# chengl7-lab/scape

Hardware: AMD Instinct MI355X
Metric: UTR regions/sec (infer_pa EM to convergence), 50k UTRs x 2k reads synthetic (higher is better)
Workload: dtype f64; 1 GPU; 50k-UTR synthetic stream x 2000 reads, K=1..10 x 10 restarts; step = one resident batch of 512 UTRs per GPU; reads_per_utr=2000, k_cap=10, n_frag_max=1469, re_run_mode=False, rng_mode=per_utr, parallelism=utr-shard x1

## Files before the change

### scape_amd/csrc/em_lockstep.inc

```

#define MT_RB 1
#define MT_ROWS (64 * MT_RB)
#define MT_NC 32
#define MT_PITCH (MT_NC + 2)
#define MT_VPITCH (MT_NC + 2)
#define MT_MAXJ 64
#ifndef EM_DEPTH
#define EM_DEPTH 3
#endif
static_assert(EM_DEPTH >= 1 && EM_DEPTH <= 8, "column slots per job");
#ifndef MT_DV1
#define MT_DV1 1
#endif

#ifndef MT_DEEP
#define MT_DEEP 2
#endif
#define CNT_SLAB 4
#define CNT_EXEC (4 + 64)
#define CNT_MSTEP_TENSOR (4 + 2 * 64)
#define CNT_MSTEP_VREQ (4 + 3 * 64)
#define CNT_MSTEP_VUNI (4 + 4 * 64)
static_assert(MT_ROWS == TILE_ROWS, "tile height must match k_tile_extent / the host tables");
static_assert(MT_MAXJ <= 64, "the per-pass job setup gives one job to each lane of one wavefront");

struct EmState {
    int32_t *ia, *ib, *sia, *sib;
    double *ws, *slw;
    double *lb, *ell;
    int32_t *nlb, *status;
    unsigned long long *pend;
    int32_t *rd_k, *rd_lo, *rd_hi, *rd_m;
    int32_t *rd_n0, *rd_n1;
    double *rd_lw, *rd_sv;
    double *rd_fl;
    double *V;
    double *Vsuf;
    const int64_t *voff;
    double *pt_score;
    int32_t *pt_row;
    const int64_t *ptoff;
};

__device__ __forceinline__ double d_wave_allsum(double v) {
#pragma unroll
    for (int off = 32; off > 0; off >>= 1) v += __shfl_xor(v, off, 64);
    return v;
}

#ifndef ESTEP_EXP_GROUP
#define ESTEP_EXP_GROUP 1
#endif
struct EstepNext {
    int status;
    int nlb;
    int pub_k;
    int k_next;
};

template <int CA, int CX, int NW = 1>
__device__ __forceinline__ EstepNext estep_body(
    const UtrDesc *__restrict__ descs, const DevParams &P, const double *__restrict__ cnt,
    const double *__restrict__ M, int kmax, const int32_t *__restrict__ job_utr,
    const int32_t *__restrict__ job_K, const int32_t *__restrict__ job_fixed,
    const int32_t *__restrict__ a_in, const int32_t *__restrict__ b_in,
    const double *__restrict__ ws_in, const int8_t *__restrict__ k_arr, const EmState &S,
    int32_t *__restrict__ a_out, int32_t *__restrict__ b_out, double *__restrict__ ws_out,
    double *__restrict__ bic_out, int32_t *__restrict__ nlb_out, double *__restrict__ lb_out,
    unsigned long long *__restrict__ counters, int launch, int slot, int depth, int job, int lane, int status,
    unsigned long long *s_roff, double *s_lwc, double *s_wsum ,
    const double2 *s_exptab , int wave = 0, double *s_xz = nullptr ,
    double *s_tot = nullptr ) {
    constexpr int CMAX = CA;
#ifdef ESTEP_STAMPS
    const unsigned long long st0 = __builtin_amdgcn_s_memtime();
#define ESTEP_STAMP(v) const unsigned long long v = __builtin_amdgcn_s_memtime()
#else
#define ESTEP_STAMP(v)
#endif
    const bool lead = (NW == 1) || wave == 0;
    const int nround = P.nround, B = P.B;
    const int u_job = job_utr[job];
    const int K = (CX > 0) ? CX - 1 : job_K[job], C = K + 1;
    const bool fixed = job_fixed[job] != 0;
    int32_t *ia = S.ia + (size_t)job * kmax, *ib = S.ib + (size_t)job * kmax;
    int32_t *sia = S.sia + (size_t)job * kmax, *sib = S.sib + (size_t)job * kmax;
    double *ws = S.ws + (size_t)job * (kmax + 1), *slw = S.slw + (size_t)job * (kmax + 1);
    const bool r0 = launch == 0 && slot == 0;
    const bool resolve = slot == 0 && launch > 0;
    const size_t col0 = (size_t)job * depth, col = col0 + slot;
    int pre_m[EM_DEPTH], pre_lo[EM_DEPTH], pre_hi[EM_DEPTH], pre_k[EM_DEPTH];
    int64_t pre_ptoff[EM_DEPTH];
    double pre_fl[EM_DEPTH];
    bool rdm = false;
#pragma unroll
    for (int q = 0; q < EM_DEPTH; ++q) {
        const bool on = resolve && q < depth;
        pre_m[q] = on ? S.rd_m[col0 + q] : 0;
        pre_lo[q] = on ? S.rd_lo[col0 + q] : 0;
        pre_hi[q] = on ? S.rd_hi[col0 + q] : 0;
        pre_k[q] = on ? S.rd_k[col0 + q] : 0;
        pre_ptoff[q] = on ? S.ptoff[col0 + q] : 0;
        pre_fl[q] = on ? S.rd_fl[col0 + q] : 0.0;
        rdm = rdm || pre_m[q] != 0;
    }
    const int64_t pre_voff = S.voff[col];
    const int k_lane = (lane < nround) ? (int)k_arr[(size_t)job * nround + lane] : 0;
    const double lb_prev = r0 ? SENT : S.lb[job];
    const int nlb_prev = r0 ? 0 : S.nlb[job];
    auto k_of_round = [&](int i) {
        const int ii = min(i, nround - 1);
        return (nround <= 64) ? __shfl(k_lane, ii, 64) : (int)k_arr[(size_t)job * nround + ii];
    };
    const int k_now = k_of_round(nlb_prev);
    const int k_next = __builtin_amdgcn_readfirstlane(k_of_round(nlb_prev + 1));
    double my_ws = 0.0, my_slw = 0.0;
    int my_ia = 0, my_ib = 0, my_sia = 0, my_sib = 0;
    if (lane < C) {
        my_ws = r0 ? ws_in[(size_t)job * (kmax + 1) + lane] : ws[lane];
        if (!r0) my_slw = slw[lane];
        if (lane < K) {
            my_ia = r0 ? a_in[(size_t)job * kmax + lane] : ia[lane];
            my_ib = r0 ? b_in[(size_t)job * kmax + lane] : ib[lane];
            my_sia = r0 ? my_ia : sia[lane];
// ... 34 lines not shown
                ia[lane] = sia[lane] = my_ia;
                ib[lane] = sib[lane] = my_ib;
            }
        }
        if (lane == 0) {
            S.lb[job] = SENT;
            S.nlb[job] = 0;
            S.ell[job] = 0.0;
        }
    }
    int upd_k[EM_DEPTH], upd_a[EM_DEPTH], upd_b[EM_DEPTH];
#pragma unroll
    for (int q = 0; q < EM_DEPTH; ++q) {
        upd_k[q] = -1;
        upd_a[q] = upd_b[q] = 0;
        if (pre_m[q]) {
            double best = pt_best[q];
            int best_r = pt_best_r[q];
#pragma unroll
            for (int off = 32; off > 0; off >>= 1) {
                const double ob = __shfl_xor(best, off, 64);
                const int orr = __shfl_xor(best_r, off, 64);
                if (ob > best || (ob == best && orr < best_r)) {
                    best = ob;
                    best_r = orr;
                }
            }
            upd_k[q] = pre_k[q];
            upd_a[q] = best_r / B;
            upd_b[q] = best_r - upd_a[q] * B;
            if (lead && lane == 0) {
                ia[upd_k[q]] = upd_a[q];
                ib[upd_k[q]] = upd_b[q];
            }
            if (lane == upd_k[q]) {
                my_ia = upd_a[q];
                my_ib = upd_b[q];
            }
        }
    }
    if (slot == 0 && lead && lane == 0 && (r0 || rdm))
        for (int q = 0; q < depth; ++q) S.rd_m[col0 + q] = 0;
    auto cur_ia = [&](int i) {
        int v = ia[i];
#pragma unroll
        for (int q = 0; q < EM_DEPTH; ++q) v = (i == upd_k[q]) ? upd_a[q] : v;
        return v;
    };
    auto cur_ib = [&](int i) {
        int v = ib[i];
#pragma unroll
        for (int q = 0; q < EM_DEPTH; ++q) v = (i == upd_k[q]) ? upd_b[q] : v;
        return v;
    };

    if (status == 1 || nlb_prev >= nround) {
        if (lead && lane == 0) {
            const int n_lb = S.nlb[job];
            bic_out[job] = d_bic(S.ell[job], K, N);
            nlb_out[job] = n_lb;
            int idx[CMAX];
            for (int i = 0; i < K; ++i) idx[i] = i;
            for (int i = 1; i < K; ++i) {
                const int v = idx[i];
                int j = i - 1;
                while (j >= 0 && cur_ia(idx[j]) > cur_ia(v)) {
                    idx[j + 1] = idx[j];
                    --j;
                }
                idx[j + 1] = v;
            }
            for (int i = 0; i < K; ++i) {
                a_out[(size_t)job * kmax + i] = cur_ia(idx[i]);
                b_out[(size_t)job * kmax + i] = cur_ib(idx[i]);
                ws_out[(size_t)job * (kmax + 1) + i] = ws[idx[i]];
            }
            ws_out[(size_t)job * (kmax + 1) + K] = ws[K];
            for (int i = K; i < kmax; ++i) {
                a_out[(size_t)job * kmax + i] = -1;
                b_out[(size_t)job * kmax + i] = -1;
                ws_out[(size_t)job * (kmax + 1) + i + 1] = 0.0;
            }
            S.status[job] = 2;
            atomicAdd(&counters[0], (unsigned long long)n_lb);
            atomicAdd(&counters[2], (unsigned long long)n_lb * (unsigned long long)N * (unsigned long long)C);
        }
        return EstepNext{2, nlb_prev, -1, 0};
    }

    if (lead && lane == 0) atomicAdd(&counters[CNT_EXEC + (job & 63)], 1ull);
    const int k = k_now;
    const double wk_old = __shfl(my_ws, k, 64);
    const double slw_k = d_logw(wk_old);
    const int sia_k = (k < K) ? __shfl(my_ia, k, 64) : 0;
    const int sib_k = (k < K) ? __shfl(my_ib, k, 64) : 0;
    const int ia_km1 = __shfl(my_ia, max(k - 1, 0), 64), ia_kp1 = __shfl(my_ia, min(k + 1, 63), 64);
    if (lead && lane == 0) {
        slw[k] = slw_k;
        if (k < K) {
            sia[k] = sia_k;
            sib[k] = sib_k;
        }
    }
    if (lead && lane < CMAX) {
        const int c = lane;
        int sa = 0, sb = 0;
        double lw_c = 0.0;
        if (c < C) {
            if (c == k) {
                lw_c = slw_k;
                sa = sia_k;
                sb = sib_k;
            } else {
                lw_c = my_slw;
                sa = my_sia;
                sb = my_sib;
            }
        }
        s_roff[c] = (c < K) ? ((unsigned long long)sa * B + sb) * Np : 0ull;
        s_lwc[c] = (c < K) ? lw_c : lw_c + d.unif_ll;
    }
    __syncthreads();
    double *Vj = S.V + pre_voff;

    ESTEP_STAMP(st1);
    double tot_w[CMAX], t_sumk = 0.0, t_ell = 0.0, t_ent = 0.0;
    int nz_lo = 0x7fffffff, nz_hi = -1;
    bool mod = false;
    if constexpr (NW == 1) {
        for (int pass = 0; pass < 2; ++pass) {
    #pragma unroll
            for (int c = 0; c < CMAX; ++c) s_wsum[c * 64 + lane] = 0.0;
            double sumk = 0.0, ell = 0.0, ent = 0.0;
            nz_lo = 0x7fffffff;
            nz_hi = -1;
            double mcur[CMAX], ccur = 0.0;
            auto fetch = [&](int n, double (&m)[CMAX], double &cn) {
                const bool ok = n < N;
                cn = ok ? cu[n] : 0.0;
    #pragma unroll
                for (int c = 0; c < CMAX; ++c) m[c] = (ok && c < K) ? Mu[s_roff[c] + n] : 0.0;
            };
            fetch(lane, mcur, ccur);
    #pragma unroll
            for (int c = 0; c < CMAX; ++c) asm volatile("" : "+v"(mcur[c]));
            asm volatile("" : "+v"(ccur));
            for (int n = lane; n < Np; n += 64) {
                double mnext[CMAX], cnext;
                fetch(n + 64, mnext, cnext);
                double vkn = 0.0;
                if (n < N) {
                    const double cn = ccur;
                    auto lzv = [&](int c) { return (c < K) ? s_lwc[c] + mcur[c] : s_lwc[c]; };
                    double mx = 0.0;
    #pragma unroll
                    for (int c = 0; c < CMAX; ++c) {
                        if (c < C) {
                            const double v = lzv(c);
                            mx = (c == 0 || v > mx) ? v : mx;
                        }
                    }
                    double z[CMAX];
                    unsigned long long live = 0ull;
#if ESTEP_EXP_GROUP >= 2
    #pragma unroll
                    for (int c = 0; c < CMAX; c += ESTEP_EXP_GROUP) {
// ... 300 lines not shown
        S.lb[job] = lb_new;
        S.status[job] = status_new;
        S.rd_m[col] = has_m ? 1 : 0;
        if (has_m) {
            const int lo = (k == 0) ? 0 : ia_km1;
            const int hi = (k == K - 1) ? d.T - 1 : ia_kp1;
            S.rd_k[col] = k;
            S.rd_lo[col] = lo * B;
            S.rd_hi[col] = (hi + 1) * B;
            S.rd_lw[col] = d_logw(wk_new);
            S.rd_sv[col] = sv;
            S.rd_fl[col] = d_logw(wk_new) * sv + SENT * v_total;
            S.rd_n0[col] = (nz_hi >= 0) ? nz_lo : 0;
            S.rd_n1[col] = (nz_hi >= 0) ? nz_hi + 1 : 0;
            atomicAdd(&counters[CNT_SLAB + (job & 63)], (unsigned long long)(hi + 1 - lo) * B * (unsigned long long)N);
        }
    }
#ifdef ESTEP_STAMPS
    if (NW == 1 && lane == 0) {
        const unsigned long long st5 = __builtin_amdgcn_s_memtime();
        unsigned long long *sp = counters + 4 + 5 * 64;
        atomicAdd(&sp[0], st1 - st0);
        atomicAdd(&sp[1], st2 - st1);
        atomicAdd(&sp[2], st3 - st2);
        atomicAdd(&sp[3], st4 - st3);
        atomicAdd(&sp[4], st5 - st4);
        atomicAdd(&sp[7], 1ull);
    }
#endif
#undef ESTEP_STAMP
    return EstepNext{status_new, nlb_prev + 1, has_m ? k : -1, k_next};
}

#define ESTEP_ARGS(ROUND, STATUS) descs, P, cnt, M, kmax, job_utr, job_K, job_fixed, a_in, b_in, ws_in, k_arr, S, a_out, \
                   b_out, ws_out, bic_out, nlb_out, lb_out, counters, ROUND, slot, depth, job, lane, STATUS, s_roff, s_lwc, s_wsum, s_exptab
#define ESTEP_CASE(C, ROUND, STATUS) \
    case C: nx = estep_body<C, C, ESTEP_NW>(ESTEP_ARGS(ROUND, STATUS) ESTEP_EXTRA); break;
#define ESTEP_DISPATCH(CM, ROUND, STATUS)                                                         \
    do {                                                                                          \
        if constexpr (CM <= 16) {                                                                 \
            const int c_exact = job_K[job] + 1;                                                   \
            if constexpr (CM >= 16) {                                                             \
                if (c_exact > 12) {                                                               \
                    switch (c_exact) {                                                            \
                        ESTEP_CASE(13, ROUND, STATUS) ESTEP_CASE(14, ROUND, STATUS)               \
                        ESTEP_CASE(15, ROUND, STATUS)                                             \
                        default: nx = estep_body<16, 16, ESTEP_NW>(ESTEP_ARGS(ROUND, STATUS) ESTEP_EXTRA); break;            \
                    }                                                                             \
                    break;                                                                        \
                }                                                                                 \
            }                                                                                     \
            if constexpr (CM >= 12) {                                                             \
                if (c_exact > 8) {                                                                \
                    switch (c_exact) {                                                            \
                        ESTEP_CASE(9, ROUND, STATUS) ESTEP_CASE(10, ROUND, STATUS)                \
                        ESTEP_CASE(11, ROUND, STATUS)                                             \
                        default: nx = estep_body<12, 12, ESTEP_NW>(ESTEP_ARGS(ROUND, STATUS) ESTEP_EXTRA); break;            \
                    }                                                                             \
                    break;                                                                        \
                }                                                                                 \
            }                                                                                     \
            if constexpr (CM >= 8) {                                                              \
                if (c_exact > 4) {                                                                \
                    switch (c_exact) {                                                            \
                        ESTEP_CASE(5, ROUND, STATUS) ESTEP_CASE(6, ROUND, STATUS)                 \
                        ESTEP_CASE(7, ROUND, STATUS)                                              \
                        default: nx = estep_body<8, 8, ESTEP_NW>(ESTEP_ARGS(ROUND, STATUS) ESTEP_EXTRA); break;              \
                    }                                                                             \
                    break;                                                                        \
                }                                                                                 \
            }                                                                                     \
            switch (c_exact) {                                                                    \
                ESTEP_CASE(1, ROUND, STATUS) ESTEP_CASE(2, ROUND, STATUS) ESTEP_CASE(3, ROUND, STATUS) \
                default: nx = estep_body<4, 4, ESTEP_NW>(ESTEP_ARGS(ROUND, STATUS) ESTEP_EXTRA); break;                      \
            }                                                                                     \
        } else {                                                                                  \
            nx = estep_body<CM, 0, ESTEP_NW>(ESTEP_ARGS(ROUND, STATUS) ESTEP_EXTRA);                                       \
        }                                                                                         \
    } while (0)

__host__ __device__ inline bool em_run_ahead_stops(int status, int nlb, int nround, int k_next, unsigned long long pend) {
    return status != 0 || nlb >= nround || (pend & (7ull << k_next)) != 0ull;
}
#define ESTEP_NW 1
#ifndef ESTEP_WPS
#define ESTEP_WPS 3
#endif
#define ESTEP_EXTRA
template <int CMAX>
__global__ __launch_bounds__(64, (CMAX > 12 ? 2 : ESTEP_WPS)) void k2_estep(
    const UtrDesc *__restrict__ descs, DevParams P, const double *__restrict__ cnt,
    const double *__restrict__ M, int kmax, const int32_t *__restrict__ job_utr,
    const int32_t *__restrict__ job_K, const int32_t *__restrict__ job_fixed,
    const int32_t *__restrict__ a_in, const int32_t *__restrict__ b_in,
    const double *__restrict__ ws_in, const int8_t *__restrict__ k_arr, EmState S,
    int32_t *__restrict__ a_out, int32_t *__restrict__ b_out, double *__restrict__ ws_out,
    double *__restrict__ bic_out, int32_t *__restrict__ nlb_out, double *__restrict__ lb_out,
    unsigned long long *__restrict__ counters, int launch, int slot, int depth, const int32_t *__restrict__ job_list,
    int n_jobs) {
    const int chunk = (n_jobs + 7) >> 3;
    const int jidx = (int)(blockIdx.x & 7) * chunk + (int)(blockIdx.x >> 3);
    if (jidx >= n_jobs) return;
    const int job = job_list[jidx];
    const int lane = threadIdx.x;
    const int status = (launch == 0 && slot == 0) ? 0 : S.status[job];
    if (status == 2) return;
    unsigned long long pend = 0ull;
    if (slot > 0) {
        pend = S.pend[job];
        if (!(pend & 1ull)) return;
        pend &= ~1ull;
    }
    __shared__ unsigned long long s_roff[CMAX];
    __shared__ double s_lwc[CMAX];
    __shared__ double s_wsum[CMAX * 64];
    __shared__ double2 s_exptab[128];
    d_load_exptab(s_exptab, lane, 64);
    EstepNext nx;
    ESTEP_DISPATCH(CMAX, launch, status);
    if (depth > 1 && lane == 0) {
        if (nx.pub_k >= 0) pend |= 2ull << nx.pub_k;
        const bool stop = em_run_ahead_stops(nx.status, nx.nlb, P.nround, nx.k_next, pend) || job_fixed[job] != 0;
        S.pend[job] = pend | (stop ? 0ull : 1ull);
    }
}

template <int CMAX>
__global__ __launch_bounds__(64, (CMAX > 12 ? 2 : 3)) void k2_estep_all_rounds(
    const UtrDesc *__restrict__ descs, DevParams P, const double *__restrict__ cnt,
    const double *__restrict__ M, int kmax, const int32_t *__restrict__ job_utr,
    const int32_t *__restrict__ job_K, const int32_t *__restrict__ job_fixed,
    const int32_t *__restrict__ a_in, const int32_t *__restrict__ b_in,
    const double *__restrict__ ws_in, const int8_t *__restrict__ k_arr, EmState S,
    int32_t *__restrict__ a_out, int32_t *__restrict__ b_out, double *__restrict__ ws_out,
    double *__restrict__ bic_out, int32_t *__restrict__ nlb_out, double *__restrict__ lb_out,
    unsigned long long *__restrict__ counters, const int32_t *__restrict__ job_list, int n_jobs) {
    const int chunk = (n_jobs + 7) >> 3;
    const int jidx = (int)(blockIdx.x & 7) * chunk + (int)(blockIdx.x >> 3);
    if (jidx >= n_jobs) return;
    const int job = job_list[jidx];
    const int lane = threadIdx.x;
    __shared__ unsigned long long s_roff[CMAX];
    __shared__ double s_lwc[CMAX];
    __shared__ double s_wsum[CMAX * 64];
    __shared__ double2 s_exptab[128];
    d_load_exptab(s_exptab, lane, 64);
    for (int round = 0; round <= P.nround; ++round) {
        const int status = (round == 0) ? 0 : S.status[job];
        if (status == 2) return;
        constexpr int slot = 0, depth = 1;
        EstepNext nx;
        ESTEP_DISPATCH(CMAX, round, status);
        (void)nx;
        __threadfence();
        __syncthreads();
    }
}
#undef ESTEP_NW
#undef ESTEP_EXTRA
#define ESTEP_NW 4
#define ESTEP_EXTRA , wave, s_xz, s_tot
template <int CMAX>
__global__ __launch_bounds__(256, 1) void k2_estep_cs(
    const UtrDesc *__restrict__ descs, DevParams P, const double *__restrict__ cnt,
    const double *__restrict__ M, int kmax, const int32_t *__restrict__ job_utr,
    const int32_t *__restrict__ job_K, const int32_t *__restrict__ job_fixed,
// ... 313 lines not shown
```

### scape_amd/csrc/scape_hip.hip

```cpp
#include <hip/hip_runtime.h>

#include <algorithm>
#include <atomic>
#include <cmath>
#include <cstdint>
#include <cstdio>
#include <cstdlib>
#include <cstring>
#include <memory>
#include <string>
#include <type_traits>
#include <chrono>
#include <utility>
#include <vector>

#include "scape_hip.h"

#define SENT SCAPE_SENT
#define PI_REF 3.141592653589793
#define PITCH 16
#define TILE_ROWS 64

static thread_local std::string g_err;
static int fail(const std::string &msg) {
// ... 557 lines not shown
            if (c < C) {
                lz[c] = (c < K) ? slw[c] + Mu[roff[c] + n] : slw[c] + d.unif_ll;
                mx = (c == 0 || lz[c] > mx) ? lz[c] : mx;
            } else {
                lz[c] = 0.0;
            }
        }
#pragma unroll
        for (int c = 0; c < CMAX; ++c) z[c] = (c < C) ? d_exp_nonpos((lz[c] - mx) * cn, s_exptab) : 0.0;
        const double s = d_np_sum<CMAX>(z, C);
        int best = 0;
        double bz = 0.0;
#pragma unroll
        for (int c = 0; c < CMAX; ++c) {
            const double zc = z[c] / s;
            if (c < C && (c == 0 || zc > bz)) {
                bz = zc;
                best = c;
            }
        }
        labels[d.bin_off + n] = best;
    }
}

struct DevBuf {
    void *p = nullptr;
    size_t cap = 0;
    DevBuf() = default;
    DevBuf(const DevBuf &) = delete;
    DevBuf &operator=(const DevBuf &) = delete;
    ~DevBuf() { release(); }
    int ensure(size_t bytes) {
        if (bytes <= cap && p) return 0;
        const bool regrow = p != nullptr || (bytes > ((size_t)1 << 30) && bytes <= ((size_t)48 << 30));
        if (p) {
            (void)hipFree(p);
            p = nullptr;
            cap = 0;
        }
        if (bytes == 0) bytes = 16;
        size_t want = regrow ? bytes + bytes / 8 : bytes;
        if (hipMalloc(&p, want) != hipSuccess) {
            (void)hipGetLastError();
            p = nullptr;
            want = bytes;
            HIPCHK(hipMalloc(&p, want));
        }
        cap = want;
        return 0;
    }
    void release() {
        if (p) (void)hipFree(p);
        p = nullptr;
        cap = 0;
    }
    template <typename T>
    T *as() const {
        return reinterpret_cast<T *>(p);
    }
};
static_assert(!std::is_copy_constructible<DevBuf>::value && !std::is_copy_assignable<DevBuf>::value,
              "a copy of a DevBuf would free its memory twice");

struct StreamDrain {
    hipStream_t stream;
    bool armed;
    explicit StreamDrain(hipStream_t s, bool a = true) : stream(s), armed(a) {}
    StreamDrain(const StreamDrain &) = delete;
    StreamDrain &operator=(const StreamDrain &) = delete;
    int wait() { armed = false; HIPCHK(hipStreamSynchronize(stream)); return 0; }
    ~StreamDrain() { if (armed) (void)hipStreamSynchronize(stream); }
};

struct EventPair {
    hipEvent_t a, b;
};

struct ReportState;

struct EmBufs {
    DevBuf ia, ib, sia, sib, ws, slw, lb, ell, nlb, status, pend, rd_k, rd_lo, rd_hi, rd_m, rd_n0, rd_n1, rd_lw, rd_sv, rd_fl, V, Vsuf,
        voff, pt_score, pt_row, ptoff;
    DevBuf ujoff, ujlist, active, elist, dbg;
    int ensure(size_t nj, size_t nc, size_t kmax, size_t n_utr, size_t vtot, size_t pttot) {
        return ia.ensure(nj * kmax * 4) || ib.ensure(nj * kmax * 4) || sia.ensure(nj * kmax * 4) || sib.ensure(nj * kmax * 4) ||
               ws.ensure(nj * (kmax + 1) * 8) || slw.ensure(nj * (kmax + 1) * 8) || lb.ensure(nj * 8) || ell.ensure(nj * 8) ||
               nlb.ensure(nj * 4) || status.ensure(nj * 4) || pend.ensure(nj * 8) || rd_k.ensure(nc * 4) || rd_lo.ensure(nc * 4) ||
               rd_hi.ensure(nc * 4) || rd_m.ensure(nc * 4) || rd_n0.ensure(nc * 4) || rd_n1.ensure(nc * 4) ||
               rd_lw.ensure(nc * 8) || rd_sv.ensure(nc * 8) || rd_fl.ensure(nc * 8) || V.ensure(vtot * 8) || Vsuf.ensure((vtot / 16 + nc + 1) * 8) ||
               voff.ensure(nc * 8) || pt_score.ensure(pttot * 8) || pt_row.ensure(pttot * 4) || ptoff.ensure(nc * 8) ||
               ujoff.ensure((n_utr + 1) * 8) || ujlist.ensure(nc * 4) || active.ensure(n_utr * 4) || elist.ensure(nj * 4);
    }
    EmState state() const {
        return EmState{ia.as<int32_t>(), ib.as<int32_t>(), sia.as<int32_t>(), sib.as<int32_t>(), ws.as<double>(), slw.as<double>(),
                       lb.as<double>(), ell.as<double>(), nlb.as<int32_t>(), status.as<int32_t>(), pend.as<unsigned long long>(),
                       rd_k.as<int32_t>(),
                       rd_lo.as<int32_t>(), rd_hi.as<int32_t>(), rd_m.as<int32_t>(), rd_n0.as<int32_t>(), rd_n1.as<int32_t>(),
                       rd_lw.as<double>(), rd_sv.as<double>(), rd_fl.as<double>(), V.as<double>(), Vsuf.as<double>(), voff.as<int64_t>(),
                       pt_score.as<double>(), pt_row.as<int32_t>(), ptoff.as<int64_t>()};
    }
};

static int to_dev(hipStream_t s, const DevBuf &d, const void *src, size_t bytes) {
    HIPCHK(hipMemcpyAsync(d.p, src, bytes, hipMemcpyHostToDevice, s));
    return 0;
}
static int to_host(hipStream_t s, void *dst, const DevBuf &d, size_t bytes) {
    HIPCHK(hipMemcpyAsync(dst, d.p, bytes, hipMemcpyDeviceToHost, s));
    return 0;
}

struct JobBufs {
    DevBuf utr, K, fixed, a, b, ws, karr, ao, bo, wso, bic, nlb, lb, sel, lbsel;
};
struct LabelBufs {
    DevBuf utr, K, a, b, ws, labels;
};

struct BatchShape {
    int n_utr = 0, T_max = 0, Np_max = 0, W_max = 1, tiles_max_all = 1;
    int64_t n_bins = 0;
    std::vector<UtrDesc> h_desc;
    size_t at_total = 0, m_total = 0, tiles_total = 0, n_theta_total = 0, mlog_total = 0, n_logbins = 0;
    bool pb_slide = false;
};
struct BatchPlan : BatchShape {
    std::vector<int32_t> loglist, logbin_utr;
};

struct BatchState : BatchShape {
    DevParams prm;
    bool loaded = false, built = false;
    bool build_unchecked = false;
    int pb_form = 0;
    int last_em_jobs = 0;
    DevBuf d_x, d_l, d_r, d_pa, d_cnt, d_theta, d_desc, d_loglist, d_AT, d_V, d_M, d_tile_nend;
    DevBuf d_tbi, d_tbG, d_tbpm, d_mlog, d_logbin;
    JobBufs job;
    LabelBufs lab;
    EmBufs em;
};

#define N_COUNTERS (4 + 5 * 64 + 16 + 48)
struct scape_hip_ctx {
    int device = 0;
    std::atomic<bool> busy{false};
    hipStream_t stream = nullptr;
    char name[256] = {0};
    std::unique_ptr<BatchState> batch;
    DevBuf d_err, d_counters;
    std::vector<EventPair> ev[6];
    double ms_acc[6] = {0, 0, 0, 0, 0, 0};
    int n_acc[6] = {0, 0, 0, 0, 0, 0};
    unsigned long long h_counters[3] = {0, 0, 0};
    unsigned long long h_traffic[4] = {0, 0, 0, 0};
    ReportState *rep = nullptr;
};

static int ev_begin(scape_hip_ctx *c, int which) {
    EventPair e;
    HIPCHK(hipEventCreate(&e.a));
    HIPCHK(hipEventCreate(&e.b));
    HIPCHK(hipEventRecord(e.a, c->stream));
    c->ev[which].push_back(e);
    return 0;
}
static int ev_end(scape_hip_ctx *c, int which) {
    HIPCHK(hipEventRecord(c->ev[which].back().b, c->stream));
    return 0;
}
static int ev_collect(scape_hip_ctx *c) {
    HIPCHK(hipStreamSynchronize(c->stream));
    const bool trace = getenv("SCAPE_HIP_ROUND_TRACE") != nullptr;
    for (int w = 0; w < 6; ++w) {
        int i = 0;
        for (auto &e : c->ev[w]) {
            float ms = 0;
            HIPCHK(hipEventElapsedTime(&ms, e.a, e.b));
            if (trace && w >= 4) fprintf(stderr, "[trace] kind %d launch %d %.4f ms\n", w, i, ms);
            ++i;
            c->ms_acc[w] += ms;
            c->n_acc[w] += 1;
// ... 94 lines not shown
    const dim3 by_alpha((unsigned)(((b.n_utr + 7) / 8) * 8 * b.T_max));
    if (ch.form == 0) {
#ifdef SCAPE_HIP_TOOLS
        const char *pe = getenv("SCAPE_HIP_PB_PROBE");
        const int probe = pe ? atoi(pe) : 0;
#else
        const int probe = 0;
#endif
        if (b.prm.B <= 16)
            hipLaunchKernelGGL(k_phase_b<16>, by_alpha, dim3(256), ch.lds, c->stream, desc, b.prm, r, pa, theta, loglist, AT, V, M,
                               ch.Wmax, all_log, c->d_err.as<int>(), b.n_utr, b.T_max, tile_nend, probe);
        else
            hipLaunchKernelGGL(k_phase_b<1>, by_alpha, dim3(256), ch.lds, c->stream, desc, b.prm, r, pa, theta, loglist, AT, V, M,
                               ch.Wmax, all_log, c->d_err.as<int>(), b.n_utr, b.T_max, tile_nend, probe);
        HIPCHK(hipGetLastError());
        return 0;
    }
    const bool slide = ch.form == 2;
    hipLaunchKernelGGL(k_pb_tables<16>, dim3((unsigned)b.T_max, (unsigned)b.n_utr), dim3(PB_TAB_THREADS), ch.lds_t, c->stream, desc,
                       b.prm, theta, ch.Wmax, ch.WP, tbi, tbG, tbpm, c->d_err.as<int>(), b.T_max, slide ? nullptr : loglist, AT, M, mlog,
                       tile_nend);
    HIPCHK(hipGetLastError());
    if (slide) {
        if (b.n_logbins) {
            hipLaunchKernelGGL(k_pb_logcol, dim3((unsigned)b.n_logbins), dim3(256), ch.lds_c, c->stream, desc, b.prm, theta, loglist,
                               b.d_logbin.as<int32_t>(), AT, tbi, tbG, M, mlog, tile_nend, ch.Wmax);
            HIPCHK(hipGetLastError());
        }
        const int blocks_max = (b.Np_max + 63) / 64;
        hipLaunchKernelGGL(k_pb_slide, dim3((unsigned)(((b.n_utr + 7) / 8) * 8 * blocks_max)), dim3(256), ch.lds_s, c->stream, desc,
                           b.prm, r, pa, loglist, V, M, mlog, ch.WP, tbi, tbpm, b.n_utr, blocks_max, tile_nend);
    } else {
        hipLaunchKernelGGL(k_phase_b_lin, by_alpha, dim3(256), ch.lds_l, c->stream, desc, b.prm, r, pa, loglist, V, M, mlog, ch.WP, tbi,
                           tbpm, b.n_utr, b.T_max, tile_nend);
    }
    HIPCHK(hipGetLastError());
    return 0;
}

static int check_err_flag(scape_hip_ctx *c, const char *what) {
    int flag = 0;
    HIPCHK(hipMemcpyAsync(&flag, c->d_err.p, sizeof(int), hipMemcpyDeviceToHost, c->stream));
    HIPCHK(hipStreamSynchronize(c->stream));
    if (flag) return fail(std::string(what) + ": device-side consistency check failed (flag " + std::to_string(flag) + ")");
    return 0;
}

static int finish_build(scape_hip_ctx *c) {
    BatchState *b = c->batch.get();
    if (!b || !b->build_unchecked) return 0;
    b->build_unchecked = false;
    b->built = check_err_flag(c, "batch_build") == 0;
    return !b->built;
}

using EstepClasses = std::integer_sequence<int, 4, 8, 12, 16, 24, 32, 64>;
using WideClasses = std::integer_sequence<int, 4, 8, 12, 16>;
using LabelClasses = std::integer_sequence<int, 8, 16, 32, 64>;

template <int... Cs>
constexpr int last_class(std::integer_sequence<int, Cs...>) {
    int last = 0;
    ((last = Cs), ...);
    return last;
}
static_assert(last_class(EstepClasses{}) == SCAPE_MAX_K + 1 && last_class(LabelClasses{}) == SCAPE_MAX_K + 1,
              "the largest class holds the largest kmax a call may have");
constexpr int WIDE_MAX_COLUMNS = last_class(WideClasses{});

template <int... Cs, typename F>
static bool with_column_class(std::integer_sequence<int, Cs...>, int columns, F &&f) {
    return ((columns <= Cs && (f(std::integral_constant<int, Cs>()), true)) || ...);
}

struct EmPlan {
    std::vector<int64_t> ujoff, voff, ptoff;
    std::vector<int32_t> ujlist, active, elist;
    size_t vtot = 0, pttot = 0;
    int depth = 1;
    int tiles_max = 1, max_cols_utr = 1;
    bool any_m = false;
};

static EmPlan em_plan(const std::vector<UtrDesc> &h_desc, int B, size_t nj, const int32_t *job_utr, const int32_t *job_fixed,
                      bool size_order, int depth) {
    EmPlan p;
    const int n_utr = (int)h_desc.size();
    p.depth = depth;
    p.ujoff.assign(n_utr + 1, 0);
    p.ujlist.resize(nj * depth);
    for (size_t j = 0; j < nj; ++j) p.ujoff[job_utr[j] + 1] += depth;
    for (int u = 0; u < n_utr; ++u) p.ujoff[u + 1] += p.ujoff[u];
    {
        std::vector<int64_t> fill(p.ujoff.begin(), p.ujoff.end() - 1);
        for (size_t j = 0; j < nj; ++j)
            for (int q = 0; q < depth; ++q) p.ujlist[fill[job_utr[j]]++] = (int32_t)(j * depth + q);
    }
    for (int u = 0; u < n_utr; ++u)
        if (p.ujoff[u + 1] > p.ujoff[u]) p.active.push_back(u);
    if (size_order)
        std::stable_sort(p.active.begin(), p.active.end(), [&](int32_t a, int32_t b) {
            const UtrDesc &da = h_desc[a], &db = h_desc[b];
            return (int64_t)da.T * da.Np > (int64_t)db.T * db.Np;
        });
    const int n_active = (int)p.active.size();
    for (int u : p.active) {
        p.max_cols_utr = std::max<int>(p.max_cols_utr, (int)(p.ujoff[u + 1] - p.ujoff[u]));
        p.tiles_max = std::max(p.tiles_max, (h_desc[u].T * B + MT_ROWS - 1) / MT_ROWS);
    }
    p.voff.resize(nj * depth);
    p.ptoff.resize(nj * depth);
    for (size_t j = 0; j < nj; ++j) {
        const UtrDesc &d = h_desc[job_utr[j]];
        for (int q = 0; q < depth; ++q) {
            p.voff[j * depth + q] = (int64_t)p.vtot;
            p.ptoff[j * depth + q] = (int64_t)p.pttot;
            p.vtot += (size_t)d.Np;
            p.pttot += (size_t)((d.T * B + MT_ROWS - 1) / MT_ROWS);
        }
        p.any_m = p.any_m || job_fixed[j] == 0;
    }
    p.elist.reserve(nj);
    auto jobs_of = [&](int u) {
        for (int64_t q = p.ujoff[u]; q < p.ujoff[u + 1]; q += depth) p.elist.push_back(p.ujlist[q] / depth);
    };
    if (size_order && n_active >= 8) {
        for (int x = 0; x < 8; ++x)
            for (int k = x; k < n_active; k += 8) jobs_of(p.active[k]);
    } else {
        for (int u = 0; u < n_utr; ++u) jobs_of(u);
    }
    return p;
}

struct EmSwitches {
    bool size_order, debug, fine, mstep_v2, mstep_v3;
    int split_maxtiles, wide_maxjobs;
    int depth;
};
static EmSwitches em_switches() {
    const char *env_m = getenv("SCAPE_HIP_MSTEP"), *env_r = getenv("SCAPE_HIP_SPLIT_MAXTILES"), *env_w = getenv("SCAPE_HIP_WIDE_MAXJOBS");
    EmSwitches s;
    s.size_order = !getenv("SCAPE_HIP_NO_SIZE_ORDER");
    s.debug = getenv("SCAPE_HIP_DEBUG") != nullptr;
    s.fine = getenv("SCAPE_HIP_ROUND_TIMING") != nullptr;
    s.mstep_v2 = env_m && strcmp(env_m, "v2") == 0;
    s.mstep_v3 = env_m && strcmp(env_m, "v3") == 0;
    s.split_maxtiles = env_r ? atoi(env_r) : 1024;
    s.wide_maxjobs = env_w ? atoi(env_w) : 1024;
    const char *env_d = getenv("SCAPE_HIP_EM_DEPTH");
    s.depth = std::min(EM_DEPTH, std::max(1, env_d ? atoi(env_d) : EM_DEPTH));
    return s;
}

struct EmKernels {
    bool wide;
    bool job_split;
    bool ring_mstep;
    bool multi_mstep;
};
static bool em_wide(const EmSwitches &sw, int n_jobs, int kmax) {
    const bool wide = n_jobs <= sw.wide_maxjobs && kmax + 1 <= WIDE_MAX_COLUMNS;
    return wide;
}

static int em_depth(const std::vector<UtrDesc> &h_desc, int B, const EmSwitches &sw, int n_jobs, int kmax, const int32_t *job_utr,
                    const int32_t *job_fixed) {
    bool any_m = false;
    size_t v1 = 0, pt1 = 0;
    std::vector<int> per_utr(h_desc.size(), 0);
    int max_jobs_utr = 1;
    for (int j = 0; j < n_jobs; ++j) {
        const UtrDesc &d = h_desc[job_utr[j]];
        any_m = any_m || job_fixed[j] == 0;
        v1 += (size_t)d.Np;
        pt1 += (size_t)((d.T * B + MT_ROWS - 1) / MT_ROWS);
        max_jobs_utr = std::max(max_jobs_utr, ++per_utr[job_utr[j]]);
    }
    if (!any_m || em_wide(sw, n_jobs, kmax)) return 1;
    int depth = sw.depth;
    while (depth > 1 && ((size_t)max_jobs_utr * depth > 1024 || v1 * depth * 8 >= ((size_t)1 << 31) || pt1 * depth >= ((size_t)1 << 31)))
        --depth;
    return depth;
}

static int em_choose(const EmPlan &p, const EmSwitches &sw, int n_jobs, int kmax, EmKernels &k) {
    k.wide = em_wide(sw, n_jobs, kmax);
    k.job_split = (long long)p.active.size() * p.tiles_max <= sw.split_maxtiles;
    k.ring_mstep = !sw.mstep_v2 && p.vtot * 8 < ((size_t)1 << 31);
    k.multi_mstep = k.ring_mstep && !k.job_split && !sw.debug && p.pttot < ((size_t)1 << 31) && !sw.mstep_v3;
    if (k.multi_mstep && M4_LDS_BYTES > 64 * 1024)
        HIPCHK(hipFuncSetAttribute(reinterpret_cast<const void *>(k4_mstep), hipFuncAttributeMaxDynamicSharedMemorySize, M4_LDS_BYTES));
    if (k.ring_mstep && M3_LDS_BYTES > 64 * 1024)
        HIPCHK(hipFuncSetAttribute(reinterpret_cast<const void *>(k3_mstep), hipFuncAttributeMaxDynamicSharedMemorySize, M3_LDS_BYTES));
    return 0;
}

static int em_upload(scape_hip_ctx *c, const EmPlan &p, size_t nj, int kmax) {
    EmBufs &e = c->batch->em;
    const size_t nc = nj * p.depth;
    if (e.ensure(nj, nc, kmax, c->batch->n_utr, p.vtot, p.pttot)) return 1;
    StreamDrain drain(c->stream);
    hipStream_t s = c->stream;
    if (to_dev(s, e.elist, p.elist.data(), nj * 4) || (!p.active.empty() && to_dev(s, e.active, p.active.data(), p.active.size() * 4)) ||
        to_dev(s, e.voff, p.voff.data(), nc * 8) || to_dev(s, e.ptoff, p.ptoff.data(), nc * 8) ||
        to_dev(s, e.ujoff, p.ujoff.data(), p.ujoff.size() * 8) || to_dev(s, e.ujlist, p.ujlist.data(), nc * 4))
        return 1;
    return drain.wait();
}

template <typename Kernel, typename... Round>
static void launch_estep(scape_hip_ctx *c, Kernel kernel, unsigned threads, const EmState &S, int kmax, const int32_t *job_list,
                         int n_jobs, Round... round) {
    const BatchState &b = *c->batch;
    const JobBufs &j = b.job;
    hipLaunchKernelGGL(kernel, dim3((unsigned)(((n_jobs + 7) / 8) * 8)), dim3(threads), 0, c->stream, b.d_desc.as<UtrDesc>(),
                       b.prm, b.d_cnt.as<double>(), b.d_M.as<double>(), kmax, j.utr.as<int32_t>(), j.K.as<int32_t>(),
                       j.fixed.as<int32_t>(), j.a.as<int32_t>(), j.b.as<int32_t>(), j.ws.as<double>(), j.karr.as<int8_t>(), S,
                       j.ao.as<int32_t>(), j.bo.as<int32_t>(), j.wso.as<double>(), j.bic.as<double>(), j.nlb.as<int32_t>(),
                       j.lb.as<double>(), c->d_counters.as<unsigned long long>(), round..., job_list, n_jobs);
}

template <typename Kernel>
static void launch_estep_slots(scape_hip_ctx *c, Kernel kernel, const EmState &S, int kmax, const int32_t *job_list, int n_jobs,
                               int r, int slots, int depth) {
    for (int slot = 0; slot < slots; ++slot) launch_estep(c, kernel, 64, S, kmax, job_list, n_jobs, r, slot, depth);
}

template <typename Kernel, typename... Tail>
static void launch_mstep(scape_hip_ctx *c, Kernel kernel, unsigned grid_y, unsigned threads, size_t lds, const EmState &S,
                         int n_active, int extent, Tail... tail) {
    const BatchState &b = *c->batch;
    hipLaunchKernelGGL(kernel, dim3((unsigned)(((n_active + 7) / 8) * 8 * extent), grid_y), dim3(threads), lds, c->stream,
                       b.d_desc.as<UtrDesc>(), b.prm, b.d_M.as<double>(), b.em.active.as<int32_t>(), n_active, extent,
                       b.em.ujoff.as<int64_t>(), b.em.ujlist.as<int32_t>(), S.V, S.Vsuf, S.voff, S.rd_m, S.rd_lo, S.rd_hi,
                       S.rd_lw, S.rd_sv, S.rd_n0, S.rd_n1, S.ptoff, S.pt_score, S.pt_row, b.d_tile_nend.as<int32_t>(),
                       c->d_counters.as<unsigned long long>(), tail...);
}

static int em_debug_round(scape_hip_ctx *c, int r, int nround) {
    unsigned long long *dbg = c->batch->em.dbg.as<unsigned long long>();
    if (r < nround) {
        unsigned long long shard[64], tb = 0;
        HIPCHK(hipMemcpy(shard, c->d_counters.as<unsigned long long>() + CNT_MSTEP_TENSOR, sizeof(shard), hipMemcpyDeviceToHost));
        for (int i = 0; i < 64; ++i) tb += shard[i];
        fprintf(stderr, "[em bytes %d] %llu\n", r, tb);
    }
    if (r == 0 || r == 10 || r == 25 || r == nround - 1) {
        unsigned long long h[24];
        HIPCHK(hipMemcpy(h, dbg, sizeof(h), hipMemcpyDeviceToHost));
        fprintf(stderr, "[em round %d] job-halfchunks own-support %llu, union %llu, padded to groups %llu; sorted-by-n1 groups %llu\n", r, h[16], h[17], h[18], h[19]);
        fprintf(stderr, "[em round %d] tiles %llu active %llu sum_cnt %llu passes %llu | G-hist:", r, h[0], h[1], h[2], h[3]);
        for (int i = 4; i < 16; ++i) fprintf(stderr, " %llu", h[i]);
        fprintf(stderr, "\n");
        HIPCHK(hipMemsetAsync(dbg, 0, 24 * sizeof(unsigned long long), c->stream));
    }
    return 0;
}

static int em_rounds(scape_hip_ctx *c, const EmPlan &p, const EmSwitches &sw, const EmKernels &k, int n_jobs, int kmax) {
    EmBufs &em = c->batch->em;
    const EmState S = em.state();
    const int nround = c->batch->prm.nround, n_active = (int)p.active.size();
    const int32_t *jl = em.elist.as<int32_t>();
    unsigned long long *dbg = nullptr;
    if (sw.debug) {
        if (em.dbg.ensure(24 * sizeof(unsigned long long))) return 1;
        dbg = em.dbg.as<unsigned long long>();
        HIPCHK(hipMemsetAsync(dbg, 0, 24 * sizeof(unsigned long long), c->stream));
    }
    if (!p.any_m) {
        if (sw.fine && ev_begin(c, 4)) return 1;
        if (!with_column_class(EstepClasses{}, kmax + 1, [&](auto cm) {
                launch_estep(c, k2_estep_all_rounds<decltype(cm)::value>, 64, S, kmax, em.ujlist.as<int32_t>(), n_jobs);
            }))
            return fail("no E-step kernel for kmax " + std::to_string(kmax));
        HIPCHK(hipGetLastError());
        if (sw.fine && ev_end(c, 4)) return 1;
        return 0;
    }
    const int jobs_per_pass = k.job_split ? 16 : MT_MAXJ;
    const unsigned psplit = k.job_split ? (unsigned)std::min(64, (p.max_cols_utr + 15) / 16) : 1u;
    unsigned long long executed_prev = 0;
    const int probe_mask = (n_jobs >= 8192 && p.depth == 1) ? 7 : 3;
    for (int r = 0; r <= nround; ++r) {
        if (sw.fine && ev_begin(c, 4)) return 1;
        const bool launched =
            k.wide ? with_column_class(WideClasses{}, kmax + 1, [&](auto cm) {
                         launch_estep(c, k2_estep_cs<decltype(cm)::value>, 256, S, kmax, jl, n_jobs, r);
                     })
                   : with_column_class(EstepClasses{}, kmax + 1, [&](auto cm) {
                         launch_estep_slots(c, k2_estep<decltype(cm)::value>, S, kmax, jl, n_jobs, r, r < nround ? p.depth : 1, p.depth);
                     });
        if (!launched) return fail("no E-step kernel for kmax " + std::to_string(kmax));
        HIPCHK(hipGetLastError());
        if (sw.fine && ev_end(c, 4)) return 1;
        if (r < nround) {
            if (sw.fine && ev_begin(c, 5)) return 1;
            if (k.multi_mstep)
                launch_mstep(c, k4_mstep, 1u, 64 * M4_NW, M4_LDS_BYTES, S, n_active, (p.tiles_max + M4_TPW - 1) / M4_TPW);
            else if (k.ring_mstep)
                launch_mstep(c, k3_mstep, psplit, 256, M3_LDS_BYTES, S, n_active, p.tiles_max, jobs_per_pass, dbg);
            else
                launch_mstep(c, k2_mstep, psplit, 256, 0, S, n_active, p.tiles_max, jobs_per_pass, dbg);
            c->h_traffic[3] += 1;
            HIPCHK(hipGetLastError());
            if (sw.fine && ev_end(c, 5)) return 1;
        }
        if (r < nround && (r & probe_mask) == probe_mask) {
            unsigned long long executed = 0, shard[64];
            HIPCHK(hipMemcpyAsync(shard, c->d_counters.as<unsigned long long>() + CNT_EXEC, sizeof(shard),
                                  hipMemcpyDeviceToHost, c->stream));
            HIPCHK(hipStreamSynchronize(c->stream));
            for (int i = 0; i < 64; ++i) executed += shard[i];
            if (executed == executed_prev) break;
            executed_prev = executed;
        }
        if (sw.debug && em_debug_round(c, r, nround)) return 1;
    }
    return 0;
}

static int em_lockstep(scape_hip_ctx *c, int n_jobs, int kmax, const int32_t *job_utr, const int32_t *job_fixed) {
    const EmSwitches sw = em_switches();
    const BatchState &b = *c->batch;
    const int depth = em_depth(b.h_desc, b.prm.B, sw, n_jobs, kmax, job_utr, job_fixed);
    const EmPlan plan = em_plan(b.h_desc, b.prm.B, (size_t)n_jobs, job_utr, job_fixed, sw.size_order, depth);
    EmKernels kernels;
    if (em_choose(plan, sw, n_jobs, kmax, kernels) || em_upload(c, plan, (size_t)n_jobs, kmax)) return 1;
    return em_rounds(c, plan, sw, kernels, n_jobs, kmax);
}

static int batch_plan(const scape_hip_params &p, int n_utr, const int64_t *bin_off, const int64_t *theta_off,
                      const double *all_theta, const double *r, const double *pa, const double *utr_L, const double *min_theta,
                      const double *unif_ll, BatchPlan &out) {
    BatchPlan s;
    double bmax = p.betas[0];
    for (int j = 1; j < p.n_beta; ++j) bmax = std::max(bmax, p.betas[j]);
    s.h_desc.assign(n_utr, UtrDesc());
    bool slide = p.n_beta <= 16;
    for (int u = 0; u < n_utr; ++u) {
        UtrDesc &d = s.h_desc[u];
        const int64_t N = bin_off[u + 1] - bin_off[u], T = theta_off[u + 1] - theta_off[u];
        if (N < 1 || T < 1 || N > (1 << 26) || T > 65535) return fail("UTR " + std::to_string(u) + ": bad n_frag / n_theta");
        const double *th = all_theta + theta_off[u];
        for (int64_t i = 1; i < T; ++i)
            if (!(th[i] >= th[i - 1])) return fail("UTR " + std::to_string(u) + ": all_theta must be ascending");
        d.bin_off = bin_off[u];
        d.theta_off = theta_off[u];
        d.N = (int)N;
        d.Np = round_up((int)N, PITCH);
        d.T = (int)T;
        d.at_off = (int64_t)s.at_total;
        d.m_off = (int64_t)s.m_total;
        d.log_off = (int64_t)s.loglist.size();
        d.tile_off = (int64_t)s.tiles_total;
        const int nt = (int)((T * p.n_beta + TILE_ROWS - 1) / TILE_ROWS);
        s.tiles_total += (size_t)nt;
        s.tiles_max_all = std::max(s.tiles_max_all, nt);
        for (int64_t n = 0; n < N; ++n)
            if (!std::isnan(pa[bin_off[u] + n]) || !std::isnan(r[bin_off[u] + n])) s.loglist.push_back((int32_t)n);
        d.n_log = (int)(s.loglist.size() - (size_t)d.log_off);
        d.mlog_off = (int64_t)s.mlog_total;
        if (d.n_log > 0 && d.n_log <= PB_LOGCAP) s.mlog_total += (size_t)T * p.n_beta * d.n_log;
        s.logbin_utr.insert(s.logbin_utr.end(), (size_t)d.n_log, (int32_t)u);
        d.c_lo = 1;
        d.c_hi = 0;
        const double step0 = (T > 1) ? th[1] - th[0] : 0.0;
        bool uni = step0 > 0.0;
        for (int64_t i = 0; i < T && uni; ++i) uni = std::floor(th[i]) == th[i] && (i == 0 || th[i] - th[i - 1] == step0);
        if (uni) {
            const int rmax = (int)std::floor(3 * bmax / step0) + 1;
            d.c_lo = rmax + 1;
            d.c_hi = (int)T - 2 - rmax;
        }
        if (d.c_lo > d.c_hi) slide = false;
        d.unif_ll = unif_ll[u];
        d.L = utr_L[u];
        d.min_theta = min_theta[u];
        s.at_total += (size_t)T * d.Np;
        s.m_total += (size_t)T * p.n_beta * d.Np;
        s.T_max = std::max(s.T_max, d.T);
        s.Np_max = std::max(s.Np_max, d.Np);
        s.W_max = std::max(s.W_max, max_window(th, d.T, bmax));
    }
    s.n_utr = n_utr;
    s.n_bins = bin_off[n_utr];
    s.n_theta_total = (size_t)theta_off[n_utr];
    s.n_logbins = s.logbin_utr.size();
    s.pb_slide = slide && s.W_max <= 4 * PB_STEPS && s.T_max <= 4096;
    out = std::move(s);
    return 0;
}

static int em_jobs_check(const BatchState &b, int n_jobs, int kmax, const int32_t *job_utr, const int32_t *job_K,
                         const int32_t *job_fixed, const int32_t *alpha_idx, const int32_t *beta_idx, const int8_t *k_arr) {
    const int nround = b.prm.nround, B = b.prm.B;
    for (int j = 0; j < n_jobs; ++j) {
        const int u = job_utr[j], K = job_K[j];
// ... 504 lines not shown
```

Before: 3349 UTRs/s.

## Compact converged EM jobs and UTRs between rounds to shrink launch grids

```diff
diff --git a/scape_amd/csrc/em_lockstep.inc b/scape_amd/csrc/em_lockstep.inc
--- a/scape_amd/csrc/em_lockstep.inc
+++ b/scape_amd/csrc/em_lockstep.inc
@@ -16,6 +16,7 @@
 #ifndef MT_DEEP
 #define MT_DEEP 2
 #endif
+#define CNT_DONE 3
 #define CNT_SLAB 4
 #define CNT_EXEC (4 + 64)
 #define CNT_MSTEP_TENSOR (4 + 2 * 64)
@@ -40,6 +41,7 @@
     double *pt_score;
     int32_t *pt_row;
     const int64_t *ptoff;
+    int32_t *u_done;
 };
 
 __device__ __forceinline__ double d_wave_allsum(double v) {
@@ -240,6 +242,8 @@
                 ws_out[(size_t)job * (kmax + 1) + i + 1] = 0.0;
             }
             S.status[job] = 2;
+            atomicAdd(&counters[CNT_DONE], 1ull);
+            if (S.u_done) atomicAdd(&S.u_done[u_job], 1);
             atomicAdd(&counters[0], (unsigned long long)n_lb);
             atomicAdd(&counters[2], (unsigned long long)n_lb * (unsigned long long)N * (unsigned long long)C);
         }
@@ -706,6 +710,67 @@
 __host__ __device__ inline bool em_run_ahead_stops(int status, int nlb, int nround, int k_next, unsigned long long pend) {
     return status != 0 || nlb >= nround || (pend & (7ull << k_next)) != 0ull;
 }
+__host__ inline int em_slots_needed(int max_k_live, int depth) {
+    return std::min(depth, max_k_live <= 2 ? 1 : max_k_live == 3 ? 2 : depth);
+}
+__host__ inline bool em_shrink_due(long long listed, long long live, int pct) {
+    return live > 0 && live < listed && live * 100 <= listed * pct;
+}
+__host__ __device__ inline int em_shrink_pos(int base, const int *wave_cnt, int wave, unsigned long long mask, int lane) {
+    int off = base;
+    for (int w = 0; w < wave; ++w) off += wave_cnt[w];
+    unsigned long long below = mask & ((1ull << lane) - 1ull);
+    int n = 0;
+    for (; below; below &= below - 1) ++n;
+    return off + n;
+}
+
+#define EM_SHRINK_THREADS 1024
+#ifndef EM_SHRINK_AT
+#define EM_SHRINK_AT 50
+#endif
+__global__ __launch_bounds__(EM_SHRINK_THREADS) void k_em_shrink(int32_t *elist, int n_list, const int32_t *__restrict__ status,
+                                                                 const int32_t *__restrict__ job_K, const int32_t *__restrict__ job_fixed,
+                                                                 int32_t *active, int n_active, const int32_t *__restrict__ u_done,
+                                                                 const int64_t *__restrict__ ujob_off, int depth, int32_t *__restrict__ out) {
+    __shared__ int s_cnt[EM_SHRINK_THREADS / 64];
+    __shared__ int s_k;
+    const int tid = threadIdx.x, lane = tid & 63, wave = tid >> 6;
+    if (tid == 0) s_k = 0;
+    int k_live = 0;
+    auto compact = [&](int32_t *list, int n, auto keep) {
+        int base = 0;
+        for (int i0 = 0; i0 < n; i0 += EM_SHRINK_THREADS) {
+            const int i = i0 + tid;
+            int32_t v = 0;
+            bool kp = false;
+            if (i < n) {
+                v = list[i];
+                kp = keep(v);
+            }
+            const unsigned long long mask = __ballot(kp);
+            if (lane == 0) s_cnt[wave] = __popcll(mask);
+            __syncthreads();
+            if (kp) list[em_shrink_pos(base, s_cnt, wave, mask, lane)] = v;
+            for (int w = 0; w < EM_SHRINK_THREADS / 64; ++w) base += s_cnt[w];
+            __syncthreads();
+        }
+        return base;
+    };
+    const int jobs = compact(elist, n_list, [&](int32_t j) {
+        const bool live = status[j] != 2;
+        if (live && job_fixed[j] == 0) k_live = max(k_live, job_K[j]);
+        return live;
+    });
+    const int utrs = compact(active, n_active, [&](int32_t u) { return (int64_t)u_done[u] * depth < ujob_off[u + 1] - ujob_off[u]; });
+    if (k_live) atomicMax(&s_k, k_live);
+    __syncthreads();
+    if (tid == 0) {
+        out[0] = jobs;
+        out[1] = utrs;
+        out[2] = s_k;
+    }
+}
 #define ESTEP_NW 1
 #ifndef ESTEP_WPS
 #define ESTEP_WPS 3
diff --git a/scape_amd/csrc/scape_hip.hip b/scape_amd/csrc/scape_hip.hip
--- a/scape_amd/csrc/scape_hip.hip
+++ b/scape_amd/csrc/scape_hip.hip
@@ -663,6 +663,7 @@
     DevBuf ia, ib, sia, sib, ws, slw, lb, ell, nlb, status, pend, rd_k, rd_lo, rd_hi, rd_m, rd_n0, rd_n1, rd_lw, rd_sv, rd_fl, V, Vsuf,
         voff, pt_score, pt_row, ptoff;
     DevBuf ujoff, ujlist, active, elist, dbg;
+    DevBuf udone, shrunk;
     int ensure(size_t nj, size_t nc, size_t kmax, size_t n_utr, size_t vtot, size_t pttot) {
         return ia.ensure(nj * kmax * 4) || ib.ensure(nj * kmax * 4) || sia.ensure(nj * kmax * 4) || sib.ensure(nj * kmax * 4) ||
                ws.ensure(nj * (kmax + 1) * 8) || slw.ensure(nj * (kmax + 1) * 8) || lb.ensure(nj * 8) || ell.ensure(nj * 8) ||
@@ -670,15 +671,16 @@
                rd_hi.ensure(nc * 4) || rd_m.ensure(nc * 4) || rd_n0.ensure(nc * 4) || rd_n1.ensure(nc * 4) ||
                rd_lw.ensure(nc * 8) || rd_sv.ensure(nc * 8) || rd_fl.ensure(nc * 8) || V.ensure(vtot * 8) || Vsuf.ensure((vtot / 16 + nc + 1) * 8) ||
                voff.ensure(nc * 8) || pt_score.ensure(pttot * 8) || pt_row.ensure(pttot * 4) || ptoff.ensure(nc * 8) ||
-               ujoff.ensure((n_utr + 1) * 8) || ujlist.ensure(nc * 4) || active.ensure(n_utr * 4) || elist.ensure(nj * 4);
-    }
-    EmState state() const {
+               ujoff.ensure((n_utr + 1) * 8) || ujlist.ensure(nc * 4) || active.ensure(n_utr * 4) || elist.ensure(nj * 4) ||
+               udone.ensure(n_utr * 4) || shrunk.ensure(4 * 4);
+    }
+    EmState state(bool count_done = false) const {
         return EmState{ia.as<int32_t>(), ib.as<int32_t>(), sia.as<int32_t>(), sib.as<int32_t>(), ws.as<double>(), slw.as<double>(),
                        lb.as<double>(), ell.as<double>(), nlb.as<int32_t>(), status.as<int32_t>(), pend.as<unsigned long long>(),
                        rd_k.as<int32_t>(),
                        rd_lo.as<int32_t>(), rd_hi.as<int32_t>(), rd_m.as<int32_t>(), rd_n0.as<int32_t>(), rd_n1.as<int32_t>(),
                        rd_lw.as<double>(), rd_sv.as<double>(), rd_fl.as<double>(), V.as<double>(), Vsuf.as<double>(), voff.as<int64_t>(),
-                       pt_score.as<double>(), pt_row.as<int32_t>(), ptoff.as<int64_t>()};
+                       pt_score.as<double>(), pt_row.as<int32_t>(), ptoff.as<int64_t>(), count_done ? udone.as<int32_t>() : nullptr};
     }
 };
 
@@ -939,6 +941,12 @@
     bool any_m = false;
 };
 
+static int em_tiles_max(const std::vector<UtrDesc> &h_desc, int B, const int32_t *utrs, int n) {
+    int tiles_max = 1;
+    for (int i = 0; i < n; ++i) tiles_max = std::max(tiles_max, (h_desc[utrs[i]].T * B + MT_ROWS - 1) / MT_ROWS);
+    return tiles_max;
+}
+
 static EmPlan em_plan(const std::vector<UtrDesc> &h_desc, int B, size_t nj, const int32_t *job_utr, const int32_t *job_fixed,
                       bool size_order, int depth) {
     EmPlan p;
@@ -963,8 +971,8 @@
     const int n_active = (int)p.active.size();
     for (int u : p.active) {
         p.max_cols_utr = std::max<int>(p.max_cols_utr, (int)(p.ujoff[u + 1] - p.ujoff[u]));
-        p.tiles_max = std::max(p.tiles_max, (h_desc[u].T * B + MT_ROWS - 1) / MT_ROWS);
-    }
+    }
+    p.tiles_max = em_tiles_max(h_desc, B, p.active.data(), n_active);
     p.voff.resize(nj * depth);
     p.ptoff.resize(nj * depth);
     for (size_t j = 0; j < nj; ++j) {
@@ -994,6 +1002,9 @@
     bool size_order, debug, fine, mstep_v2, mstep_v3;
     int split_maxtiles, wide_maxjobs;
     int depth;
+    bool shrink;
+    int shrink_at;
+    bool trace;
 };
 static EmSwitches em_switches() {
     const char *env_m = getenv("SCAPE_HIP_MSTEP"), *env_r = getenv("SCAPE_HIP_SPLIT_MAXTILES"), *env_w = getenv("SCAPE_HIP_WIDE_MAXJOBS");
@@ -1007,6 +1018,10 @@
     s.wide_maxjobs = env_w ? atoi(env_w) : 1024;
     const char *env_d = getenv("SCAPE_HIP_EM_DEPTH");
     s.depth = std::min(EM_DEPTH, std::max(1, env_d ? atoi(env_d) : EM_DEPTH));
+    const char *env_s = getenv("SCAPE_HIP_EM_SHRINK"), *env_a = getenv("SCAPE_HIP_EM_SHRINK_AT");
+    s.shrink = !(env_s && atoi(env_s) == 0);
+    s.shrink_at = std::min(100, std::max(1, env_a ? atoi(env_a) : EM_SHRINK_AT));
+    s.trace = getenv("SCAPE_HIP_ROUND_TRACE") != nullptr;
     return s;
 }
 
@@ -1115,11 +1130,40 @@
     return 0;
 }
 
+struct EmLive {
+    int jobs, utrs, tiles_max, slots;
+};
+static int em_shrink(scape_hip_ctx *c, const EmPlan &p, const EmSwitches &sw, int r, std::vector<int32_t> &h_active, EmLive &live) {
+    const BatchState &b = *c->batch;
+    const EmBufs &em = b.em;
+    hipLaunchKernelGGL(k_em_shrink, dim3(1), dim3(EM_SHRINK_THREADS), 0, c->stream, em.elist.as<int32_t>(), live.jobs,
+                       em.status.as<int32_t>(), b.job.K.as<int32_t>(), b.job.fixed.as<int32_t>(), em.active.as<int32_t>(), live.utrs,
+                       em.udone.as<int32_t>(), em.ujoff.as<int64_t>(), p.depth, em.shrunk.as<int32_t>());
+    HIPCHK(hipGetLastError());
+    int32_t kept[3] = {0, 0, 0};
+    if (to_host(c->stream, kept, em.shrunk, sizeof(kept)) || to_host(c->stream, h_active.data(), em.active, (size_t)live.utrs * 4)) return 1;
+    HIPCHK(hipStreamSynchronize(c->stream));
+    if (kept[0] < 1 || kept[0] > live.jobs || kept[1] < 1 || kept[1] > live.utrs) return fail("EM shrink: inconsistent live counts");
+    const int slots = em_slots_needed(kept[2], p.depth);
+    if (sw.trace)
+        fprintf(stderr, "[shrink] pass %d jobs %d -> %d utrs %d -> %d slots %d\n", r, live.jobs, kept[0], live.utrs, kept[1], slots);
+    live = EmLive{kept[0], kept[1], em_tiles_max(b.h_desc, b.prm.B, h_active.data(), kept[1]), slots};
+    return 0;
+}
+
 static int em_rounds(scape_hip_ctx *c, const EmPlan &p, const EmSwitches &sw, const EmKernels &k, int n_jobs, int kmax) {
     EmBufs &em = c->batch->em;
-    const EmState S = em.state();
-    const int nround = c->batch->prm.nround, n_active = (int)p.active.size();
+    const bool shrinking = sw.shrink && p.any_m && !k.wide && !sw.debug;
+    const EmState S = em.state(shrinking);
+    const int nround = c->batch->prm.nround, n_active = (int)p.active.size(), n_utr = c->batch->n_utr;
     const int32_t *jl = em.elist.as<int32_t>();
+    EmLive live{n_jobs, n_active, p.tiles_max, p.depth};
+    std::vector<int32_t> h_done, h_active;
+    if (shrinking) {
+        h_done.assign(n_utr, 0);
+        h_active = p.active;
+        HIPCHK(hipMemsetAsync(em.udone.p, 0, (size_t)n_utr * 4, c->stream));
+    }
     unsigned long long *dbg = nullptr;
     if (sw.debug) {
         if (em.dbg.ensure(24 * sizeof(unsigned long long))) return 1;
@@ -1147,7 +1191,7 @@
                          launch_estep(c, k2_estep_cs<decltype(cm)::value>, 256, S, kmax, jl, n_jobs, r);
                      })
                    : with_column_class(EstepClasses{}, kmax + 1, [&](auto cm) {
-                         launch_estep_slots(c, k2_estep<decltype(cm)::value>, S, kmax, jl, n_jobs, r, r < nround ? p.depth : 1, p.depth);
+                         launch_estep_slots(c, k2_estep<decltype(cm)::value>, S, kmax, jl, live.jobs, r, r < nround ? live.slots : 1, p.depth);
                      });
         if (!launched) return fail("no E-step kernel for kmax " + std::to_string(kmax));
         HIPCHK(hipGetLastError());
@@ -1155,23 +1199,34 @@
         if (r < nround) {
             if (sw.fine && ev_begin(c, 5)) return 1;
             if (k.multi_mstep)
-                launch_mstep(c, k4_mstep, 1u, 64 * M4_NW, M4_LDS_BYTES, S, n_active, (p.tiles_max + M4_TPW - 1) / M4_TPW);
+                launch_mstep(c, k4_mstep, 1u, 64 * M4_NW, M4_LDS_BYTES, S, live.utrs, (live.tiles_max + M4_TPW - 1) / M4_TPW);
             else if (k.ring_mstep)
-                launch_mstep(c, k3_mstep, psplit, 256, M3_LDS_BYTES, S, n_active, p.tiles_max, jobs_per_pass, dbg);
+                launch_mstep(c, k3_mstep, psplit, 256, M3_LDS_BYTES, S, live.utrs, live.tiles_max, jobs_per_pass, dbg);
             else
-                launch_mstep(c, k2_mstep, psplit, 256, 0, S, n_active, p.tiles_max, jobs_per_pass, dbg);
+                launch_mstep(c, k2_mstep, psplit, 256, 0, S, live.utrs, live.tiles_max, jobs_per_pass, dbg);
             c->h_traffic[3] += 1;
             HIPCHK(hipGetLastError());
             if (sw.fine && ev_end(c, 5)) return 1;
         }
         if (r < nround && (r & probe_mask) == probe_mask) {
-            unsigned long long executed = 0, shard[64];
-            HIPCHK(hipMemcpyAsync(shard, c->d_counters.as<unsigned long long>() + CNT_EXEC, sizeof(shard),
-                                  hipMemcpyDeviceToHost, c->stream));
+            unsigned long long executed = 0, head[CNT_EXEC + 64];
+            HIPCHK(hipMemcpyAsync(head, c->d_counters.as<unsigned long long>(), sizeof(head), hipMemcpyDeviceToHost, c->stream));
+            if (shrinking && to_host(c->stream, h_done.data(), em.udone, (size_t)n_utr * 4)) return 1;
             HIPCHK(hipStreamSynchronize(c->stream));
-            for (int i = 0; i < 64; ++i) executed += shard[i];
+            for (int i = 0; i < 64; ++i) executed += head[CNT_EXEC + i];
             if (executed == executed_prev) break;
             executed_prev = executed;
+            if (shrinking) {
+                const long long live_jobs = (long long)n_jobs - (long long)head[CNT_DONE];
+                long long live_utrs = 0;
+                for (int i = 0; i < live.utrs; ++i) {
+                    const int u = h_active[i];
+                    live_utrs += (int64_t)h_done[u] * p.depth < p.ujoff[u + 1] - p.ujoff[u];
+                }
+                if ((em_shrink_due(live.jobs, live_jobs, sw.shrink_at) || em_shrink_due(live.utrs, live_utrs, sw.shrink_at)) &&
+                    em_shrink(c, p, sw, r, h_active, live))
+                    return 1;
+            }
         }
         if (sw.debug && em_debug_round(c, r, nround)) return 1;
     }
```

Result: faster. 3428 UTRs/s, median of 6 (+2.3%).
